# Sh-Anand/Raytracer-in-CPP

Measured on AMD Instinct MI355X. Metric: Mrays/s, higher is better.
Workload: dtype f32; 1 GPU; 1920x1080 depth 4 64-sample area light, cube.obj, 1 light, row stripes of 8 over 1 GPU(s); width=1920, height=1080, max_depth=4, samples=64, scene=cube.obj, parallelism=rows1, step=eager launches

## Files before the change

raytracer-in-cpp_amd/csrc/rt_kernels.hip:

```cpp
#include <hip/hip_runtime.h>

#include <cstdlib>
#include <type_traits>

#include "rt_ao_layout.hpp"
#include "rt_shadow_layout.hpp"
#include "rt_gather_layout.hpp"
#include "rt_probe_layout.hpp"
#include "rt_distance_layout.hpp"
#include "rt_hits_layout.hpp"
#include "rt_device.hpp"
#include "rt_gbuffer_layout.hpp"
#include "rt_launch.hpp"

namespace rtamd {

#define RT_WAVES 4
#define RT_STACK 128

__device__ __forceinline__ float smin(float a, float b) { return (b < a) ? b : a; }
__device__ __forceinline__ float smax(float a, float b) { return (a < b) ? b : a; }
__device__ __forceinline__ float dot3(float ax, float ay, float az, float bx, float by, float bz) {
    return ax * bx + (ay * by + az * bz);
}
__device__ __forceinline__ void normalize3(float &x, float &y, float &z) {
    const float q = x * x + (y * y + z * z);
    if (q > 0.0f) {
        const float s = sqrtf(q);
        x = x / s; y = y / s; z = z / s;
    }
}

#ifdef RT_NO_HOT_LAYOUT
#define RT_LIKELY(x) (x)
#define RT_UNLIKELY(x) (x)
#define RT_SELDOM(x) (x)
#else
#define RT_LIKELY(x) __builtin_expect(static_cast<bool>(x), true)
#define RT_UNLIKELY(x) __builtin_expect(static_cast<bool>(x), false)
#define RT_SELDOM(x) __builtin_expect_with_probability(static_cast<bool>(x), false, 0.97)
#endif

__device__ __forceinline__ void normalize3_fast(const float q, float &x, float &y, float &z) {
    float s = __builtin_amdgcn_sqrtf(q);
    const float sm = __uint_as_float(__float_as_uint(s) - 1u), sp = __uint_as_float(__float_as_uint(s) + 1u);
    const float rm = __builtin_fmaf(-sm, s, q), rp = __builtin_fmaf(-sp, s, q);
    s = rp > 0.0f ? sp : (rm <= 0.0f ? sm : s);
    float r = __builtin_amdgcn_rcpf(s);
    const float e = __builtin_fmaf(-s, r, 1.0f);
    r = __builtin_fmaf(e, r, r);
    float qx = x * r, qy = y * r, qz = z * r;
    qx = __builtin_fmaf(__builtin_fmaf(-s, qx, x), r, qx);
    qy = __builtin_fmaf(__builtin_fmaf(-s, qy, y), r, qy);
    qz = __builtin_fmaf(__builtin_fmaf(-s, qz, z), r, qz);
    x = __builtin_fmaf(__builtin_fmaf(-s, qx, x), r, qx);
    y = __builtin_fmaf(__builtin_fmaf(-s, qy, y), r, qy);
    z = __builtin_fmaf(__builtin_fmaf(-s, qz, z), r, qz);
}
__device__ __forceinline__ void normalize3_shared(float &x, float &y, float &z) {
    const float q = x * x + (y * y + z * z);
    const bool ok = (q >= 0x1p-80f) && (q <= 0x1p80f) && (fminf(fminf(fabsf(x), fabsf(y)), fabsf(z)) >= 0x1p-60f);
    if (RT_LIKELY(__ballot(!ok) == 0ull)) {
        normalize3_fast(q, x, y, z);
    } else if (q > 0.0f) {
        const float s = sqrtf(q);
        x = x / s; y = y / s; z = z / s;
    }
}
template <bool TESTED>
__device__ __forceinline__ void normalize3_shared(const float q, float &x, float &y, float &z) {
    if constexpr (TESTED) {
        normalize3_fast(q, x, y, z);
    } else {
        const bool ok = (q >= 0x1p-80f) && (q <= 0x1p80f) && (fminf(fminf(fabsf(x), fabsf(y)), fabsf(z)) >= 0x1p-60f);
        if (RT_LIKELY(__ballot(!ok) == 0ull)) {
            normalize3_fast(q, x, y, z);
        } else if (q > 0.0f) {
            const float s = sqrtf(q);
            x = x / s; y = y / s; z = z / s;
        }
    }
}

__device__ __forceinline__ uint32_t uniform_u32(uint32_t v) { return __builtin_amdgcn_readfirstlane(v); }
__device__ __forceinline__ unsigned long long uniform_u64(unsigned long long v) {
    const uint32_t lo = __builtin_amdgcn_readfirstlane(static_cast<uint32_t>(v));
    const uint32_t hi = __builtin_amdgcn_readfirstlane(static_cast<uint32_t>(v >> 32));
    return (static_cast<unsigned long long>(hi) << 32) | lo;
}
__device__ __forceinline__ uint32_t lanes_below(unsigned long long m) {
    return __builtin_amdgcn_mbcnt_hi(static_cast<uint32_t>(m >> 32), __builtin_amdgcn_mbcnt_lo(static_cast<uint32_t>(m), 0u));
}

// ... 483 lines not shown
                    RT_PROF_ADD(lane, WORK_TRI_STEPS_LANES_RAYS, 2); RT_PROF_ADD(lane, WORK_TRI_USEFUL_LANES_RAYS, 2 * __popcll(__ballot(mine)));
                    test_lane(ta);
                    test_lane(tb);
                }
                if (k < n) {
                    RT_PROF_ADD(lane, WORK_TRI_STEPS_LANES_RAYS, 1); RT_PROF_ADD(lane, WORK_TRI_USEFUL_LANES_RAYS, __popcll(__ballot(mine)));
                    test_lane(staged[k]);
                }
                if (ANY && !COUNT) {
                    mine = mine && !occluded;
                    if (__ballot(mine) == 0ull) break;
                }
            }
        }
    }
}

template <bool ANY, bool COUNT, bool STAGED = true>
__device__ __forceinline__ auto packet_walk(const DNode *__restrict__ nodes, const TriRec *__restrict__ tris,
                                            const ChunkBound *__restrict__ chunks, const uint32_t *__restrict__ leaf_chunk0,
                                            const float extent, const WaveStack stk, const int lane, const WalkCtl wc, bool in_root, const WalkRay &ray,
                                            uint32_t &cnt_box, uint32_t &cnt_ref, uint32_t &cnt_sig) {
    const RayLane R = make_ray_lane(ray, extent);
    const float ox = R.ox, oy = R.oy, oz = R.oz, idx_ = R.idx, idy_ = R.idy, idz_ = R.idz, slab_pad = R.slab_pad;
    float best_t = 3.402823466e+38f;
    int best_f = -1;
    bool occluded = false;
    int sp = 0;
    {
        unsigned long long m0 = __ballot(in_root);
        if (wc.resume) m0 &= wc.start_mask;
        if (m0 == 0ull) return walk_result<ANY>(best_t, best_f, occluded);
        if (COUNT && in_root && !wc.resume) cnt_box += 1;
        stk.node[0] = wc.resume ? wc.start_node : 0u;
        stk.mask[0] = m0;
        sp = 1;
    }
    while (sp > 0) {
        --sp;
        __builtin_amdgcn_wave_barrier();
        const uint32_t ni = uniform_u32(stk.node[sp]);
        const unsigned long long m = uniform_u64(stk.mask[sp]);
        bool mine = ((m >> lane) & 1ull) != 0ull;
        if (ANY && !COUNT) mine = mine && !occluded;
        unsigned long long live = __ballot(mine);
        if (live == 0ull) continue;
        const DNode nd = nodes[ni];
        const uint32_t cnt = nd.count_flags & 0x7fffffffu;
        if (nd.count_flags & RT_NODE_LEAF) {
            leaf_visit<ANY, COUNT, STAGED>(nd, ni, tris, chunks, leaf_chunk0, stk, lane, wc, R, live, mine, best_t, best_f, occluded, cnt_ref, cnt_sig);
        } else {
            for (uint32_t c = 0; c < cnt; ++c) {
                const uint32_t ci = nd.first + c;
                const DNode ch = nodes[ci];
                bool h = mine;
                if (!COUNT && ch.pad[1] == 0u) {
                    const float t0x = (ch.clo[0] - slab_pad - ox) * idx_, t1x = (ch.chi[0] + slab_pad - ox) * idx_;
                    const float t0y = (ch.clo[1] - slab_pad - oy) * idy_, t1y = (ch.chi[1] + slab_pad - oy) * idy_;
                    const float t0z = (ch.clo[2] - slab_pad - oz) * idz_, t1z = (ch.chi[2] + slab_pad - oz) * idz_;
                    const float tin = fmaxf(fmaxf(fminf(t0x, t1x), fminf(t0y, t1y)), fminf(t0z, t1z));
                    const float tout = fminf(fminf(fmaxf(t0x, t1x), fmaxf(t0y, t1y)), fmaxf(t0z, t1z));
                    const bool miss = (tin > tout) || (tout < -1e-3f) ||
                                      (ANY ? (tin > 0.981f) : (tin > best_t + 1e-3f * (1.0f + fabsf(best_t))));
                    RT_PROF_ADD(lane, WORK_RAY_NODE_PAIRS_CONTENT_CULLED, __popcll(__ballot(h && miss)));
                    h = h && !miss;
                    if (__ballot(h) == 0ull) continue;
                }
                h = h && box_hit_verified(ch.bmin, ox, oy, oz, ray.bx, ray.by, ray.bz, ray.brx, ray.bry, ray.brz);
                RT_PROF_ADD(lane, WORK_BOX_STEPS_STACK_WALK, 1); RT_PROF_ADD(lane, WORK_BOX_USEFUL_STACK_WALK, __popcll(__ballot(mine)));
                if (COUNT && mine) cnt_box += h ? 2u : 1u;
                const unsigned long long hm = __ballot(h);
                if (hm != 0ull) {
                    stk.node[sp] = ci;
                    stk.mask[sp] = hm;
                    ++sp;
                }
            }
        }
    }
    return walk_result<ANY>(best_t, best_f, occluded);
}


template <bool ANY, bool COUNT>
__device__ __forceinline__ auto flat_walk(const DNode &root, const TriRec *__restrict__ tris, bool in_root, const SegPacket &seg, const unsigned long long skip, const LanePlane &pl,
                                          const WalkRay &ray, uint32_t &cnt_box, uint32_t &cnt_ref) {
    const float ox = ray.ox, oy = ray.oy, oz = ray.oz, dx = ray.dx, dy = ray.dy, dz = ray.dz;
    float best_t = 3.402823466e+38f;
    int best_f = -1;
    bool occluded = false;
    if (__ballot(in_root) == 0ull) return walk_result<ANY>(best_t, best_f, occluded);
    const uint32_t cnt = root.count_flags & 0x7fffffffu;
    if (COUNT && in_root) { cnt_box += 1; cnt_ref += cnt; }
    const TriRec *__restrict__ T = tris + root.first;
    bool mine = in_root;
    auto test_one = [&](const TriRec &tr) {
        const float dn = dot3(dx, dy, dz, tr.nx, tr.ny, tr.nz);
        const float t = (tr.nA - dot3(ox, oy, oz, tr.nx, tr.ny, tr.nz)) / dn;
        const float v2x = (ox + t * dx) - tr.ax, v2y = (oy + t * dy) - tr.ay, v2z = (oz + t * dz) - tr.az;
        const float d02 = dot3(tr.e0x, tr.e0y, tr.e0z, v2x, v2y, v2z);
        const float d12 = dot3(tr.e1x, tr.e1y, tr.e1z, v2x, v2y, v2z);
        const float u = (tr.d11 * d02 - tr.d01 * d12) * tr.inv_denom;
        const float v = (tr.d00 * d12 - tr.d01 * d02) * tr.inv_denom;
        const bool ok = mine && !(ANY && (tr.flags & 1u)) && (dn != 0) && (u >= 0) && (v >= 0) && (u + v < 1) && (t > 0.00001f);
        if (ANY) {
            occluded = occluded || (ok && t < 0.98f);
        } else {
            const bool better = ok && (t < best_t || (t == best_t && static_cast<int>(tr.face) < best_f));
            best_t = better ? t : best_t;
            best_f = better ? static_cast<int>(tr.face) : best_f;
        }
    };
    if (ANY && !COUNT && seg.on) {
        unsigned long long keep = low_mask(cnt) & ~skip;
        keep &= ~__ballot(seg.prepared ? plane_rules_out_prepared(seg, pl) : plane_rules_out(seg, pl.nx, pl.ny, pl.nz, pl.nA));
        RT_PROF_ADD(threadIdx.x & 63, WORK_LEAVES_LANES_RAYS, 1); RT_PROF_ADD(threadIdx.x & 63, WORK_TRI_USEFUL_LANES_RAYS, __popcll(keep));
        while (keep != 0ull) {
            const uint32_t k0 = static_cast<uint32_t>(__builtin_ctzll(keep));
            keep &= keep - 1ull;
            if (keep != 0ull) {
                const uint32_t k1 = static_cast<uint32_t>(__builtin_ctzll(keep));
                keep &= keep - 1ull;
                TriRec ta, tb;
                tri_load_uniform_pair(T + k0, T + k1, ta, tb);
                RT_PROF_ADD(threadIdx.x & 63, WORK_TRI_STEPS_LANES_RAYS, 2);
                test_one(ta);
                test_one(tb);
            } else {
                RT_PROF_ADD(threadIdx.x & 63, WORK_TRI_STEPS_LANES_RAYS, 1);
                test_one(tri_load_uniform(T + k0));
            }
            mine = mine && !occluded;
            if (__ballot(mine) == 0ull) break;
        }
        return walk_result<ANY>(best_t, best_f, occluded);
    }
    uint32_t k = 0;
    RT_PROF_ADD(threadIdx.x & 63, WORK_LEAVES_LANES_RAYS, 1);
    for (; k + 1u < cnt; k += 2u) {
        TriRec ta, tb;
        tri_load_uniform2(T + k, ta, tb);
        RT_PROF_ADD(threadIdx.x & 63, WORK_TRI_STEPS_LANES_RAYS, 2);
        test_one(ta);
        test_one(tb);
        if (ANY && !COUNT && (k & 6u) == 6u) {
            mine = mine && !occluded;
            if (__ballot(mine) == 0ull) return walk_result<ANY>(best_t, best_f, occluded);
        }
    }
    if (k < cnt) { RT_PROF_ADD(threadIdx.x & 63, WORK_TRI_STEPS_LANES_RAYS, 1); test_one(tri_load_uniform(T + k)); }
    return walk_result<ANY>(best_t, best_f, occluded);
}

template <bool ANY, bool COUNT, bool FLAT, bool STAGED = true>
__device__ __forceinline__ auto walk(const DNode &root, const DNode *__restrict__ nodes, const TriRec *__restrict__ tris,
                                     const ChunkBound *__restrict__ chunks, const uint32_t *__restrict__ leaf_chunk0,
                                     const float extent, const WaveStack stk, const int lane, const WalkCtl wc, const LanePlane &pl, bool in_root,
                                     const WalkRay &ray, uint32_t &cnt_box, uint32_t &cnt_ref) {
    uint32_t sig_unused = 0u;
    if constexpr (FLAT) return flat_walk<ANY, COUNT>(root, tris, in_root, wc.seg, wc.skip, pl, ray, cnt_box, cnt_ref);
    else return packet_walk<ANY, COUNT, STAGED>(nodes, tris, chunks, leaf_chunk0, extent, stk, lane, wc, in_root, ray, cnt_box, cnt_ref, sig_unused);
}

template <bool COUNT>
__device__ __forceinline__ bool flat_unit_occluded(const DNode &root, const TriRec *__restrict__ tris, const SegPacket &seg, const unsigned long long skip,
                                                   const LanePlane &pl, const bool valid, const WalkRay &ray, uint32_t &cnt_box, uint32_t &cnt_ref) {
    return flat_walk<true, COUNT>(root, tris, valid && root_hit(root, ray), seg, skip, pl, ray, cnt_box, cnt_ref);
}

#ifndef RT_SHAFT_TRUNC
#define RT_SHAFT_TRUNC 0.0185f
#endif
struct ShaftLanes {
    float r[8];
    float pad;
    bool node_ok;
};

__device__ __forceinline__ ShaftLanes make_shaft_lanes(const int lane, const float hx, const float hy, const float hz, const float slx, const float sly,
                                                       const float slz, const float shx, const float shy, const float shz, const float extent,
                                                       const float trunc = 0.0f) {
    ShaftLanes SL;
    const int tk = lane & 7, proj = tk >> 1;
    const bool q1 = (tk & 1) != 0;
    const float big = fmaxf(fmaxf(fabsf(slx), fabsf(shx)), fmaxf(fabsf(sly), fabsf(shy))) + fmaxf(fabsf(slz), fabsf(shz));
    const float scale = extent + big + (fabsf(hx) + fabsf(hy) + fabsf(hz));
    SL.pad = 4e-4f * ((fmaxf(fabsf(slx), fabsf(shx)) + fmaxf(fabsf(sly), fabsf(shy)) + fmaxf(fabsf(slz), fabsf(shz))) + extent) * 1.001f;
    SL.node_ok = true;
    const float hu = proj == 1 ? hy : hx, hv = proj == 2 ? hy : hz;
    const float u0 = proj == 1 ? sly : slx, u1 = proj == 1 ? shy : shx;
    const float v0 = proj == 2 ? sly : slz, v1 = proj == 2 ? shy : shz;
    const bool ul = hu < u0, ur = hu > u1, vl = hv < v0, vr = hv > v1;
    const bool su0 = !(ul || ur), sv0 = !(vl || vr);
    const float near_u = ul ? u0 : u1, far_u = ul ? u1 : u0, near_v = vl ? v0 : v1, far_v = vl ? v1 : v0;
    const float cu = q1 ? (su0 ? u1 : (sv0 ? near_u : far_u)) : (su0 ? u0 : near_u);
    const float cv = q1 ? (sv0 ? v1 : near_v) : (sv0 ? v0 : (su0 ? near_v : far_v));
    const float mu = 0.5f * (u0 + u1) - hu, mv = 0.5f * (v0 + v1) - hv;
    const float nu = -(cv - hv), nv = cu - hu;
    const float fm = nu * mu + nv * mv;
    const float mag = fabsf(nu) + fabsf(nv);
    const bool ok = !(su0 && sv0) && (fabsf(fm) > 1e-5f * mag * scale);
    const float sgn = fm > 0.0f ? -1.0f : 1.0f;
    const float a = ok ? sgn * nu : 0.0f, b = ok ? sgn * nv : 0.0f;
    const float margin = 2e-5f * mag * scale;
    const float c = ok ? -(a * hu + b * hv) - margin : -1.0f;
    const float ax = proj == 1 ? 0.0f : a, ay = proj == 0 ? 0.0f : (proj == 1 ? a : b), az = proj == 2 ? 0.0f : b;
    SL.r[0] = fmaxf(ax, 0.0f); SL.r[1] = fminf(ax, 0.0f); SL.r[2] = fmaxf(ay, 0.0f); SL.r[3] = fminf(ay, 0.0f);
    SL.r[4] = fmaxf(az, 0.0f); SL.r[5] = fminf(az, 0.0f); SL.r[6] = c; SL.r[7] = ok ? 2.0f * margin : 3e38f;
    if (tk == 6) {
        SL.r[0] = fminf(slx, hx); SL.r[1] = fminf(sly, hy); SL.r[2] = fminf(slz, hz);
        SL.r[3] = fmaxf(shx, hx); SL.r[4] = fmaxf(shy, hy); SL.r[5] = fmaxf(shz, hz);
        if (trunc > 0.0f) {
            const float m = 1e-5f * scale;
            SL.r[0] += hx < slx ? fmaxf(trunc * (slx - hx) - m, 0.0f) : 0.0f; SL.r[3] -= hx > shx ? fmaxf(trunc * (hx - shx) - m, 0.0f) : 0.0f;
            SL.r[1] += hy < sly ? fmaxf(trunc * (sly - hy) - m, 0.0f) : 0.0f; SL.r[4] -= hy > shy ? fmaxf(trunc * (hy - shy) - m, 0.0f) : 0.0f;
            SL.r[2] += hz < slz ? fmaxf(trunc * (slz - hz) - m, 0.0f) : 0.0f; SL.r[5] -= hz > shz ? fmaxf(trunc * (hz - shz) - m, 0.0f) : 0.0f;
        }
    }
    if (tk == 7) {
        SL.r[0] = hx >= shx ? hx : -3e38f; SL.r[1] = hy >= shy ? hy : -3e38f; SL.r[2] = hz >= shz ? hz : -3e38f;
        SL.r[3] = hx <= slx ? hx : 3e38f; SL.r[4] = hy <= sly ? hy : 3e38f; SL.r[5] = hz <= slz ? hz : 3e38f;
    }
    return SL;
}

__device__ __forceinline__ void shaft_lane_test(const ShaftLanes &SL, const int tk, const float lx, const float ly, const float lz, const float hx, const float hy,
                                                const float hz, bool &near_out, bool &far_out, const bool near_box = true) {
    const float mn = __builtin_fmaf(SL.r[0], lx, __builtin_fmaf(SL.r[1], hx, __builtin_fmaf(SL.r[2], ly, __builtin_fmaf(SL.r[3], hy,
                     __builtin_fmaf(SL.r[4], lz, __builtin_fmaf(SL.r[5], hz, SL.r[6]))))));
    const float mx = __builtin_fmaf(SL.r[0], hx, __builtin_fmaf(SL.r[1], lx, __builtin_fmaf(SL.r[2], hy, __builtin_fmaf(SL.r[3], ly,
                     __builtin_fmaf(SL.r[4], hz, __builtin_fmaf(SL.r[5], lz, SL.r[6]))))));
    const bool box_out = (lx > SL.r[3]) || (hx < SL.r[0]) || (ly > SL.r[4]) || (hy < SL.r[1]) || (lz > SL.r[5]) || (hz < SL.r[2]);
    near_out = tk < 6 ? (mn > 0.0f) : (tk == 6 && near_box && box_out);
// ... 691 lines not shown
    r.lx = it.lx; r.ly = it.ly; r.lz = it.lz; r.lmode = it.lmode; r.pix = it.pix;
    r.pre = r.valid;
    return r;
}
template <bool PRIMARY, bool LENS, bool SHUTTER, bool PASS>
__device__ __forceinline__ TileRay tile_ray(const uint32_t tile, const int lane, const DFrame &F, const DCam &cam, const DShutter &shut, const DNode &root,
                                            const RayItem *__restrict__ rays_in, const ShardMap &rmap) {
    if (PRIMARY) {
        uint32_t pt = tile;
        unsigned long long lanes = ~0ull;
        if (F.tiles != nullptr) flag_tile(F, rmap, tile, pt, lanes);
        return primary_ray<LENS, SHUTTER, PASS>(pt, lanes, lane, F, cam, shut, root);
    }
    return listed_ray(tile, lane, F, rays_in, rmap);
}

__device__ __forceinline__ void finish_tile(const TileRay &r, const bool hit, const bool lit, const int best_f, const float best_t, const uint32_t tile,
                                            const int level, const int lane, const DFrame &F, ShadeItem *__restrict__ items, Control *__restrict__ ctl,
                                            float4 *__restrict__ rec, int32_t *__restrict__ out_hit, float *__restrict__ out_t) {
    if (r.valid) {
        if (!hit) rec[r.pix] = background_record();
        else if (!lit) rec[r.pix] = shadow_record();
        if (out_hit) out_hit[r.pix] = hit ? best_f : -1;
        if (out_t) out_t[r.pix] = hit ? best_t : -1.0f;
    }
    const unsigned long long lm = __ballot(lit);
    if (lm != 0ull) {
        bool fits;
        const uint32_t base = shard_reserve(ctl->n_items[level], &ctl->overflow, tile, static_cast<uint32_t>(__popcll(lm)), F.item_cap, lane, fits);
        if (lit && fits) {
            ShadeItem o;
            o.ox = r.ox; o.oy = r.oy; o.oz = r.oz; o.dx = r.dx; o.dy = r.dy; o.dz = r.dz;
            o.lx = r.lx; o.ly = r.ly; o.lz = r.lz; o.lmode = r.lmode; o.pix = r.pix; o.face = best_f; o.t = best_t;
            o.pad0 = o.pad1 = o.pad2 = 0u;
            items[base + lanes_below(lm)] = o;
        }
    }
}
template <bool PRIMARY, bool COUNT>
__device__ __forceinline__ void flush_trace_counters(Control *__restrict__ ctl, const int lane, const int level, uint32_t c_rays, uint32_t c_cull,
                                                     uint32_t c_centre, uint32_t c_box, uint32_t c_ref, const uint32_t c_outside) {
    c_rays = wave_sum(c_rays); c_cull = wave_sum(c_cull); c_centre = wave_sum(c_centre);
    c_cull += c_outside;
    if (COUNT) { c_box = wave_sum(c_box); c_ref = wave_sum(c_ref); }
    if (lane == 0) {
        if (c_rays) stat_add(ctl, (PRIMARY || level == 0) ? ST_RAYS_PRIMARY : ST_RAYS_BOUNCE, c_rays);
        if (c_cull) stat_add(ctl, ST_PIXELS_CULLED, c_cull);
        if (c_centre) stat_add(ctl, ST_RAYS_CENTRE, c_centre);
        if (COUNT) {
            if (c_box) stat_add(ctl, ST_BOX_TESTS, c_box);
            if (c_ref) stat_add(ctl, ST_LEAF_TRI_REFS, c_ref);
        }
    }
}

template <bool COUNT, bool FLAT>
__device__ __forceinline__ bool centre_lit(const DNode &root, const DNode *__restrict__ nodes, const TriRec *__restrict__ tris, const ChunkBound *__restrict__ chunks,
                                           const uint32_t *__restrict__ leaf_chunk0, const float extent, const WaveStack stk, const int lane, const DLights &L,
                                           const bool hit, const float hx, const float hy, const float hz, const uint32_t lmode, const float lx, const float ly,
                                           const float lz, uint32_t &c_centre, uint32_t &c_box, uint32_t &c_ref) {
    bool lit = false;
    const int nl_lane = lmode ? 1 : L.n_lights;
    const int nl_wave = (__ballot(hit && lmode == 0u) != 0ull) ? L.n_lights : 1;
    if (__ballot(hit) != 0ull) {
        for (int l = 0; l < nl_wave; ++l) {
            const bool act = hit && (l < nl_lane);
            float px, py, pz;
            light_point(L, l, lmode, lx, ly, lz, px, py, pz);
            c_centre += act ? 1u : 0u;
            if (COUNT && act) c_box += 1;
            const WalkRay ray = segment_ray(px, py, pz, hx, hy, hz);
            const bool occ = walk<true, COUNT, FLAT>(root, nodes, tris, chunks, leaf_chunk0, extent, stk, lane, walk_plain(), LanePlane{}, act && root_hit(root, ray), ray,
                                                     c_box, c_ref);
            lit = lit || (act && !occ);
        }
    }
    return lit;
}
__device__ __forceinline__ Hit flat_closest_hit(const DNode &root, const TriRec *__restrict__ tris, const bool active, const float ox, const float oy, const float oz,
                                                const float dx, const float dy, const float dz) {
    const WalkRay ray = trace_ray(ox, oy, oz, dx, dy, dz);
    uint32_t cu0 = 0, cu1 = 0;
    return flat_walk<false, false>(root, tris, active && root_hit(root, ray), seg_off(), 0ull, LanePlane{}, ray, cu0, cu1);
}

template <bool PRIMARY, bool COUNT, bool FLAT, bool LENS = false, bool SHUTTER = false, bool PASS = false>
__global__ __launch_bounds__(RT_WAVES * 64) void k_trace(const DNode *__restrict__ nodes, const TriRec *__restrict__ tris,
                                                          const ChunkBound *__restrict__ chunks, const uint32_t *__restrict__ leaf_chunk0,
                                                          const DScene S, const CamArg camarg, const DLights L, const DFrame F,
                                                          const int level, const int ctr_slot,
                                                          const RayItem *__restrict__ rays_in, ShadeItem *__restrict__ items,
                                                          Control *__restrict__ ctl, float4 *__restrict__ rec,
                                                          int32_t *__restrict__ out_hit, float *__restrict__ out_t) {
    __shared__ uint4 s_stage[FLAT ? 1 : RT_WAVES * RT_STAGE_TRIS * 5];
    __shared__ unsigned long long s_mask[FLAT ? 1 : RT_WAVES * RT_STACK];
    __shared__ uint32_t s_node[FLAT ? 1 : RT_WAVES * RT_STACK];
    const int lane = threadIdx.x & 63, wave = threadIdx.x >> 6;
    const WaveStack stk{s_node + (FLAT ? 0 : wave * RT_STACK), s_mask + (FLAT ? 0 : wave * RT_STACK), s_stage + (FLAT ? 0 : wave * RT_STAGE_TRIS * 5)};
    ShardMap rmap{0u, 0u, 0u, 0u};
    if (!PRIMARY) rmap = shard_map(ctl->n_rays[level], lane, 0xffffffffu, 1u, 64u);
    else if (F.tiles != nullptr) rmap = shard_map(ctl->n_flag, lane, F.tile_cap, 1u, 1u);
    uint32_t ntiles = (!PRIMARY || F.tiles != nullptr) ? rmap.total : static_cast<uint32_t>(F.tiles_x) * static_cast<uint32_t>(F.tiles_y);
    if (!PRIMARY && ntiles == 0u) return;
    const DNode root = nodes[0];
    DCam cam;
    if (PRIMARY) cam = cam_of(camarg);
    DShutter shut;
    if (PRIMARY && SHUTTER) shut = shutter_of(camarg);
    constexpr bool CULL = PRIMARY && !COUNT && !LENS && !SHUTTER && !PASS;
    const bool cull = CULL && F.cull != 0;
    CullRect crect{0, 0, 0, 0};
    bool window = false;
    uint32_t wx0 = 0, wy0 = 0, ww = 1, c_outside = 0;
    if (cull) {
        crect = cull_rect(camarg);
        if (F.nranks == 1 && out_hit == nullptr && out_t == nullptr) {
            window = true;
            const int lx0 = crect.x0 < F.width ? crect.x0 : F.width, lx1 = crect.x1 < F.width ? crect.x1 : F.width;
            int ly0 = crect.y0 - F.row0, ly1 = crect.y1 - F.row0;
            ly0 = ly0 < 0 ? 0 : (ly0 < F.local_rows ? ly0 : F.local_rows);
            ly1 = ly1 < 0 ? 0 : (ly1 < F.local_rows ? ly1 : F.local_rows);
            ntiles = 0u; c_outside = F.npix;
            if (lx0 < lx1 && ly0 < ly1) {
                const int wx1 = (lx1 + 7) / 8, wy1 = (ly1 + 7) / 8;
                wx0 = static_cast<uint32_t>(lx0 / 8); wy0 = static_cast<uint32_t>(ly0 / 8);
                ww = static_cast<uint32_t>(wx1) - wx0;
                ntiles = ww * (static_cast<uint32_t>(wy1) - wy0);
                const int px1 = wx1 * 8 < F.width ? wx1 * 8 : F.width, py1 = wy1 * 8 < F.local_rows ? wy1 * 8 : F.local_rows;
                c_outside = F.npix - static_cast<uint32_t>(px1 - static_cast<int>(wx0) * 8) * static_cast<uint32_t>(py1 - static_cast<int>(wy0) * 8);
            }
        }
    }

    uint32_t c_rays = 0, c_cull = 0, c_centre = 0, c_box = 0, c_ref = 0;
    ShardedQueue q;
    if (F.dyn_trace) q.init(ctl->queue[ctr_slot], ntiles, gridDim.x * RT_WAVES, blockIdx.x, lane);
    else q.init_static(ntiles, gridDim.x * RT_WAVES, uniform_u32(blockIdx.x * RT_WAVES + static_cast<uint32_t>(wave)), lane);
    for (uint32_t tile = 0; q.next(tile);) {
        RT_PROF_ADD(lane, WORK_UNITS, 1);
        TileRay r;
        if (PRIMARY) {
            uint32_t pt = tile;
            unsigned long long lanes = ~0ull;
            if (F.tiles != nullptr) flag_tile(F, rmap, tile, pt, lanes);
            if (window) pt = (wy0 + tile / ww) * static_cast<uint32_t>(F.tiles_x) + wx0 + tile % ww;
            if (cull && !window) {
                const int tx = static_cast<int>(pt % static_cast<uint32_t>(F.tiles_x)), ty = static_cast<int>(pt / static_cast<uint32_t>(F.tiles_x));
                if (tile_outside(F, crect, tx, ty)) {
                    const int x = tx * 8 + (lane & 7), lr = ty * 8 + (lane >> 3);
                    const bool valid = (x < F.width) && (lr < F.local_rows) && ((lanes >> lane) & 1ull) != 0ull;
                    const uint32_t pix = static_cast<uint32_t>(lr) * static_cast<uint32_t>(F.width) + static_cast<uint32_t>(x);
                    c_cull += valid ? 1u : 0u;
                    if (valid && out_hit) out_hit[pix] = -1;
                    if (valid && out_t) out_t[pix] = -1.0f;
                    continue;
                }
            }
            r = primary_ray<LENS, SHUTTER, PASS>(pt, lanes, lane, F, cam, shut, root);
            c_cull += (r.valid && !r.pre) ? 1u : 0u;
        } else {
            r = listed_ray(tile, lane, F, rays_in, rmap);
        }
        bool in_root = r.pre;
        c_rays += in_root ? 1u : 0u;
        const WalkRay ray = trace_ray(r.ox, r.oy, r.oz, r.dx, r.dy, r.dz);
        if (COUNT && in_root) c_box += 1;
        in_root = in_root && root_hit(root, ray);

        const Hit best = walk<false, COUNT, FLAT>(root, nodes, tris, chunks, leaf_chunk0, S.extent, stk, lane, walk_plain(), LanePlane{}, in_root, ray, c_box, c_ref);
        const bool hit = r.valid && found(best.face, S.n_faces);
        const float hx = r.ox + best.t * r.dx, hy = r.oy + best.t * r.dy, hz = r.oz + best.t * r.dz;
        const bool lit = centre_lit<COUNT, FLAT>(root, nodes, tris, chunks, leaf_chunk0, S.extent, stk, lane, L, hit, hx, hy, hz, r.lmode, r.lx, r.ly, r.lz,
                                                 c_centre, c_box, c_ref);

        finish_tile(r, hit, lit, best.face, best.t, tile, level, lane, F, items, ctl, rec, out_hit, out_t);
    }
    flush_trace_counters<PRIMARY, COUNT>(ctl, lane, level, c_rays, c_cull, c_centre, c_box, c_ref, (CULL && blockIdx.x == 0 && wave == 0) ? c_outside : 0u);
}


#define RT_NO_HIT_KEY 0xffffffffffffffffull

template <bool PRIMARY, bool COUNT, int STAGE, bool CONT, bool LENS = false, bool SHUTTER = false, bool PASS = false>
__global__ __launch_bounds__(RT_WAVES * 64) void k_stage(const DNode *__restrict__ nodes, const TriRec *__restrict__ tris,
                                                          const ChunkBound *__restrict__ chunks, const uint32_t *__restrict__ leaf_chunk0,
                                                          const DScene S, const CamArg camarg, const DLights L, const DFrame F,
                                                          const int level, const int lslots,
                                                          const RayItem *__restrict__ rays_in, ShadeItem *__restrict__ items,
                                                          Control *__restrict__ ctl, float4 *__restrict__ rec,
                                                          int32_t *__restrict__ out_hit, float *__restrict__ out_t,
                                                          unsigned long long *best, unsigned long long *lit, const TaskQueues Q) {
    constexpr bool CONE = CONT && STAGE < 2 && !COUNT;
    __shared__ uint4 s_stage[RT_WAVES * RT_STAGE_TRIS * 5];
    __shared__ unsigned long long s_mask[RT_WAVES * RT_STACK];
    __shared__ uint32_t s_node[RT_WAVES * RT_STACK];
    __shared__ float4 s_cone[CONE ? RT_WAVES * RT_SHAFT_TRI_REC : 1];
    const int lane = threadIdx.x & 63, wave = threadIdx.x >> 6;
    const WaveStack stk{s_node + wave * RT_STACK, s_mask + wave * RT_STACK, s_stage + wave * RT_STAGE_TRIS * 5};
    float4 *const cone_rec = s_cone + (CONE ? wave * RT_SHAFT_TRI_REC : 0);
    ShardMap rmap{0u, 0u, 0u, 0u};
    if (!PRIMARY) rmap = shard_map(ctl->n_rays[level], lane, 0xffffffffu, 1u, 64u);
    else if (F.tiles != nullptr) rmap = shard_map(ctl->n_flag, lane, F.tile_cap, 1u, 1u);
    const uint32_t ntiles = (!PRIMARY || F.tiles != nullptr) ? rmap.total : static_cast<uint32_t>(F.tiles_x) * static_cast<uint32_t>(F.tiles_y);

    uint32_t n_units = STAGE == 1 ? ntiles * static_cast<uint32_t>(lslots) : ntiles;
    ShardMap tmap{0u, 0u, 0u, 0u};
    if (CONT) {
        tmap = shard_map(ctl->n_task_tr[level][Q.q_in & 1u], lane, Q.cap / RT_LIST_SHARDS, 1u, 1u);
        n_units = tmap.total;
    }
    if (n_units == 0u) return;
    const DNode root = nodes[0];
    DCam cam;
    if (PRIMARY) cam = cam_of(camarg);
    DShutter shut;
    if (PRIMARY && SHUTTER) shut = shutter_of(camarg);
    constexpr bool CULL = PRIMARY && !COUNT && !CONT && !LENS && !SHUTTER && !PASS;
    const bool cull = CULL && F.cull != 0;
    CullRect crect{0, 0, 0, 0};
    if (cull) crect = cull_rect(camarg);

    uint32_t c_rays = 0, c_cull = 0, c_centre = 0, c_box = 0, c_ref = 0;
    ShardedQueue q;
    q.init_static(n_units, gridDim.x * RT_WAVES, uniform_u32(blockIdx.x * RT_WAVES + static_cast<uint32_t>(wave)), lane);
    for (uint32_t work = 0; q.next(work);) {
        uint32_t unit = work;
        WalkCtl wc = walk_plain();
        RT_PROF_ADD(lane, WORK_UNITS, 1);
        if (CONT) {
            uint32_t tsh, tloc, tn;
            shard_find(tmap, work, tsh, tloc, tn);
            const ContTask task = Q.tasks_in[tsh * (Q.cap / RT_LIST_SHARDS) + tloc];
            unit = uniform_u32(task.unit);
            wc.resume = true;
            wc.start_node = uniform_u32(task.node);
            wc.start_mask = uniform_u64(task.mask);
            wc.c_begin = uniform_u32(task.c_begin);
            wc.c_end = uniform_u32(task.c_end);
        }
        if (STAGE < 2 && Q.tasks_out != nullptr && Q.budget != 0u) {
            const uint32_t tsh = blockIdx.x & (RT_LIST_SHARDS - 1u), tcap = Q.cap / RT_LIST_SHARDS;
            wc.budget = Q.budget; wc.unit = unit; wc.tasks = Q.tasks_out + tsh * tcap; wc.task_count = &ctl->n_task_tr[level][Q.q_out & 1u][tsh * 16u]; wc.task_cap = tcap;
            wc.target = Q.target ? Q.target : Q.budget;
        }
        const uint32_t tile = STAGE == 1 ? unit / static_cast<uint32_t>(lslots) : unit;
        const int l = STAGE == 1 ? static_cast<int>(unit - tile * static_cast<uint32_t>(lslots)) : 0;
        if (cull) {
            const int tx = static_cast<int>(tile % static_cast<uint32_t>(F.tiles_x)), ty = static_cast<int>(tile / static_cast<uint32_t>(F.tiles_x));
            if (tile_outside(F, crect, tx, ty)) {
                const int x = tx * 8 + (lane & 7), lr = ty * 8 + (lane >> 3);
                const bool valid = (x < F.width) && (lr < F.local_rows);
                if (STAGE == 0) c_cull += valid ? 1u : 0u;
                if (STAGE == 2 && valid) {
                    const uint32_t pix = static_cast<uint32_t>(lr) * static_cast<uint32_t>(F.width) + static_cast<uint32_t>(x);
                    if (out_hit) out_hit[pix] = -1;
                    if (out_t) out_t[pix] = -1.0f;
// ... 378 lines not shown
        shard_find(imap, unit, sh, lu, n_sh);
        const uint32_t g = P == 1u ? lu : udiv(lu, P, inv_P, sh_P), pass = lu - g * P;
        const uint32_t item_i = lslots == 1 ? g : udiv(g, static_cast<uint32_t>(lslots), inv_ls, sh_ls);
        const int l = static_cast<int>(g - item_i * static_cast<uint32_t>(lslots));
        uint32_t item_at = uniform_u32(sh * item_cap + item_i);
        if (sidx != nullptr) item_at = uniform_u32(sidx[item_at]);
        if (!CONT && Q.pair_done != nullptr) {
            const size_t di = static_cast<size_t>(item_at) * static_cast<size_t>(lslots) + static_cast<size_t>(l);
            const uint32_t dw = reinterpret_cast<const uint32_t *>(Q.pair_done)[di >> 2];
            if (((dw >> (8u * static_cast<uint32_t>(di & 3u))) & 0xffu) != 0u) continue;
        }
        const ShadeItem it = items[item_at];
        uint32_t s = pass * 64u + static_cast<uint32_t>(lane);
        float fi = fi_lane + 0.5f, fj = fj_lane + 0.5f;
        float b_i0 = 0.5f, b_j0 = 0.5f, b_i1 = fi_last, b_j1 = fj_last;
        if (blocks) {
            const uint32_t bi = udiv(pass, bpr, inv_bpr, sh_bpr), bj = pass - bi * bpr;
            s = (bi * 8u + (static_cast<uint32_t>(lane) >> 3)) * vst + bj * 8u + (static_cast<uint32_t>(lane) & 7u);
            b_i0 = static_cast<float>(bi * 8u) + 0.5f; b_j0 = static_cast<float>(bj * 8u) + 0.5f;
            b_i1 = static_cast<float>(bi * 8u + 7u) + 0.5f; b_j1 = static_cast<float>(bj * 8u + 7u) + 0.5f;
            fi = (static_cast<float>(bi * 8u) + fi_lane) + 0.5f; fj = (static_cast<float>(bj * 8u) + fj_lane) + 0.5f;
        } else if (P > 1u) {
            fi = static_cast<float>(s / vst) + 0.5f; fj = static_cast<float>(s % vst) + 0.5f;
        }
        const int nl = it.lmode ? 1 : L.n_lights;
        const bool valid = s < N && l < nl;
        float hx, hy, hz;
        hit_point(it, hx, hy, hz);
        LightGrid lg = lg0;
        if (it.lmode != 0u || l != 0) {
            float px, py, pz;
            light_point(L, l, it.lmode, it.lx, it.ly, it.lz, px, py, pz);
            lg = light_grid(L, px, py, pz);
        }
        float sx, sy, sz, x0, y0, z0, x1, y1, z1;
        grid_sample(lg, fi, fj, sx, sy, sz);
        grid_sample(lg, b_i0, b_j0, x0, y0, z0);
        grid_sample(lg, b_i1, b_j1, x1, y1, z1);
        if (L.mode == RT_LIGHT_SPHERE) {
            float px, py, pz;
            light_point(L, l, it.lmode, it.lx, it.ly, it.lz, px, py, pz);
            sphere_sample(L, s, px, py, pz, sx, sy, sz);
            sphere_box(L, px, py, pz, x0, y0, z0, x1, y1, z1);
        }
        const WalkRay ray = segment_ray(sx, sy, sz, hx, hy, hz);
        const unsigned long long vis_index = (static_cast<unsigned long long>(item_at) * static_cast<unsigned long long>(lslots) + static_cast<unsigned long long>(l)) * P + pass;
        if (!CONT) c_rays += static_cast<uint32_t>(__popcll(__ballot(valid)));
        ShaftLanes SL = make_shaft_lanes(lane, hx, hy, hz, fminf(x0, x1), fminf(y0, y1), fminf(z0, z1), fmaxf(x0, x1), fmaxf(y0, y1), fmaxf(z0, z1), S.extent, RT_SHAFT_TRUNC);
        __builtin_amdgcn_wave_barrier();
        shaft_tri_store(sl.tri, lane, SL, hx, hy, hz, fminf(x0, x1), fminf(y0, y1), fminf(z0, z1), fmaxf(x0, x1), fmaxf(y0, y1), fmaxf(z0, z1));
        shaft_lanes_store(sl.shaft, lane, SL);
        __builtin_amdgcn_wave_barrier();
        ShaftCtl SC{SL.pad, true};
        SC.node_ok = __ballot(valid && !(fabsf(ray.dx) > 0.0f && fabsf(ray.dy) > 0.0f && fabsf(ray.dz) > 0.0f && fabsf(ray.dx) + fabsf(ray.dy) + fabsf(ray.dz) < 3e38f)) == 0ull;
        const RayLane R = make_ray_lane(ray, S.extent);
        bool occ = false;
        const bool tasks_on = TASKS && Q.tasks_out != nullptr && Q.budget != 0u && units < 256u * gridDim.x * RT_WAVES;
        const uint32_t tsh = blockIdx.x & (RT_LIST_SHARDS - 1u), tcap = Q.cap / RT_LIST_SHARDS;
        if (CONT) {
            const ShaftTasks TQ{nullptr, nullptr, 0u, 0u, 0u, unit};
            const unsigned long long live = t_mask & uniform_u64(vis[vis_index]);
            if (live != 0ull) {
                const DNode leaf = nodes[t_node];
                shaft_leaf<false>(t_node, uniform_u32(leaf.first), uniform_u32(leaf.count_flags) & 0x7fffffffu, uniform_u32(leaf.pad[0]), tris, chunks, lane, R, SC, TQ,
                           sl, t_cb, t_ce, live, occ);
            }
            const unsigned long long om = __ballot(valid && occ);
            if (lane == 0 && om != 0ull) atomicAnd(&vis[vis_index], ~om);
        } else {
            const DNode rootl = sl.nodes[0];
            const bool sroot = valid && root_hit(rootl, ray);
            const ShaftTasks TQ{Q.tasks_out + tsh * tcap, &ctl->n_task_sh[level][tsh * 16u], tcap, tasks_on ? Q.budget : 0u, Q.target ? Q.target : Q.budget, unit};
            shaft_walk<TASKS>(nodes, tris, chunks, stk, sl, lane, rootl, sroot, R, SC, TQ, occ);
            const unsigned long long vm = __ballot(valid && !occ);
            if (lane == 0) vis[vis_index] = vm;
        }
    }
    if (lane == 0 && c_rays) {
        stat_add(ctl, ST_RAYS_SAMPLE, c_rays);
        stat_add(ctl, ST_SAMPLE_WALKED, c_rays);
    }
}

__device__ __forceinline__ bool plane_rules_out_box(const float slx, const float sly, const float slz, const float shx, const float shy, const float shz,
                                                    const float hlx, const float hly, const float hlz, const float hhx, const float hhy, const float hhz,
                                                    const float m0, const float nx, const float ny, const float nz, const float nA) {
    const float ax = nx * slx, bx = nx * shx, ay = ny * sly, by = ny * shy, az = nz * slz, bz = nz * shz;
    const float sn_lo = fminf(ax, bx) + (fminf(ay, by) + fminf(az, bz));
    const float sn_hi = fmaxf(ax, bx) + (fmaxf(ay, by) + fmaxf(az, bz));
    const float cx = nx * hlx, dx = nx * hhx, cy = ny * hly, dy = ny * hhy, cz = nz * hlz, dz = nz * hhz;
    const float hn_lo = fminf(cx, dx) + (fminf(cy, dy) + fminf(cz, dz));
    const float hn_hi = fmaxf(cx, dx) + (fmaxf(cy, dy) + fmaxf(cz, dz));
    const float num_lo = nA - sn_hi, num_hi = nA - sn_lo;
    const float dn_lo = hn_lo - sn_hi, dn_hi = hn_hi - sn_lo;
    const float M = m0 + 2e-5f * fabsf(nA);
    const bool sane = (fabsf(nx) + fabsf(ny) + fabsf(nz) <= 4.0f) && (fabsf(nA) <= 1e30f);
    const bool opposite = (num_lo > M && dn_hi < -M) || (num_hi < -M && dn_lo > M);
    const float min_abs_num = fmaxf(num_lo, -num_hi);
    const float max_abs_dn = fmaxf(fabsf(dn_lo), fabsf(dn_hi));
    const bool beyond = (min_abs_num - M) >= 0.981f * (max_abs_dn + M);
    const float e_max = fmaxf(fabsf(hn_lo - nA), fabsf(hn_hi - nA));
    const float a_min = min_abs_num - M;
    const bool near_plane = (a_min > 0.0f) && (e_max + 2.0f * M <= 0.018f * a_min);
    return sane && (num_lo <= num_hi) && (dn_lo <= dn_hi) && (hn_lo <= hn_hi) && (opposite || beyond || near_plane);
}
__device__ __forceinline__ void shaft_inflate(ShaftLanes &SL, const int tk, const float ex, const float ey, const float ez) {
    if (tk < 6) {
        const float ax = SL.r[0] + SL.r[1], ay = SL.r[2] + SL.r[3], az = SL.r[4] + SL.r[5];
        SL.r[6] = SL.r[6] - ((fabsf(ax) * ex + fabsf(ay) * ey) + fabsf(az) * ez) * 1.0001f;
    } else if (tk == 6) {
        SL.r[0] -= ex; SL.r[1] -= ey; SL.r[2] -= ez; SL.r[3] += ex; SL.r[4] += ey; SL.r[5] += ez;
    }
}
struct ItemPlane { float a, b, c, far_margin; };
template <int PROJ, bool Q1>
__device__ __forceinline__ ItemPlane item_plane(const float hx, const float hy, const float hz, const float slx, const float sly, const float slz,
                                                const float shx, const float shy, const float shz, const float scale) {
    const float hu = PROJ == 1 ? hy : hx, hv = PROJ == 2 ? hy : hz;
    const float u0 = PROJ == 1 ? sly : slx, u1 = PROJ == 1 ? shy : shx;
    const float v0 = PROJ == 2 ? sly : slz, v1 = PROJ == 2 ? shy : shz;
    const bool ul = hu < u0, ur = hu > u1, vl = hv < v0, vr = hv > v1;
    const bool su0 = !(ul || ur), sv0 = !(vl || vr);
    const float near_u = ul ? u0 : u1, far_u = ul ? u1 : u0, near_v = vl ? v0 : v1, far_v = vl ? v1 : v0;
    const float cu = Q1 ? (su0 ? u1 : (sv0 ? near_u : far_u)) : (su0 ? u0 : near_u);
    const float cv = Q1 ? (sv0 ? v1 : near_v) : (sv0 ? v0 : (su0 ? near_v : far_v));
    const float mu = 0.5f * (u0 + u1) - hu, mv = 0.5f * (v0 + v1) - hv;
    const float nu = -(cv - hv), nv = cu - hu;
    const float fm = nu * mu + nv * mv;
    const float mag = fabsf(nu) + fabsf(nv);
    const bool ok = !(su0 && sv0) && (fabsf(fm) > 1e-5f * mag * scale);
    const float sgn = fm > 0.0f ? -1.0f : 1.0f;
    const float margin = 2e-5f * mag * scale;
    ItemPlane p;
    p.a = ok ? sgn * nu : 0.0f; p.b = ok ? sgn * nv : 0.0f;
    p.c = ok ? -(p.a * hu + p.b * hv) - margin : -1.0f;
    p.far_margin = ok ? 2.0f * margin : 3e38f;
    return p;
}
template <int PROJ>
__device__ __forceinline__ void item_plane_test(const ItemPlane &p, const float lx, const float ly, const float lz, const float hx, const float hy, const float hz,
                                                bool &near_out, bool &far_out) {
    const float ul = PROJ == 1 ? ly : lx, uh = PROJ == 1 ? hy : hx, vl = PROJ == 2 ? ly : lz, vh = PROJ == 2 ? hy : hz;
    const float ap = fmaxf(p.a, 0.0f), an = fminf(p.a, 0.0f), bp = fmaxf(p.b, 0.0f), bn = fminf(p.b, 0.0f);
    const float mn = __builtin_fmaf(ap, ul, __builtin_fmaf(an, uh, __builtin_fmaf(bp, vl, __builtin_fmaf(bn, vh, p.c))));
    const float mx = __builtin_fmaf(ap, uh, __builtin_fmaf(an, ul, __builtin_fmaf(bp, vh, __builtin_fmaf(bn, vl, p.c))));
    near_out = near_out || (mn > 0.0f);
    far_out = far_out || (mx + p.far_margin < 0.0f);
}

#ifndef RT_BEAM_BUDGET
#define RT_BEAM_BUDGET 1024
#endif
#ifndef RT_PAIR_WPE
#define RT_PAIR_WPE 6
#endif
#define RT_BEAM_REC 13

__device__ __forceinline__ bool tri_outside_beam(const float4 *rec, const TriRec &tr, const float m) {
    if (tri_outside_cone(rec, tr, m, true)) return true;
    const float4 hm = rec[8], s0 = rec[9], s1 = rec[10], h0 = rec[11], h1 = rec[12];
    return plane_rules_out_box(s0.x, s0.y, s0.z, s1.x, s1.y, s1.z, h0.x, h0.y, h0.z, h1.x, h1.y, h1.z, hm.w, tr.nx, tr.ny, tr.nz, tr.nA);
}

__device__ __forceinline__ bool beam_leaf(const uint32_t first, const uint32_t cnt, const uint32_t chunk0, const TriRec *__restrict__ tris,
                                          const ChunkBound *__restrict__ chunks, const int lane, const float4 *shaft, const float4 *rec, const ShaftCtl &SC,
                                          const bool per_item, int &budget) {
    const TriRec *__restrict__ T = tris + first;
    const ChunkBound *__restrict__ cbounds = chunks + chunk0;
    const uint32_t nchunk = (cnt + 63u) >> 6;
    const int tk = lane & 7, tc = lane >> 3;
    for (uint32_t cb0 = 0u; cb0 < nchunk; cb0 += 8u) {
        const uint32_t myc = cb0 + static_cast<uint32_t>(tc);
        const ChunkBound bd = cbounds[myc < nchunk ? myc : cb0];
        const ShaftLanes SL = shaft_lanes_load(shaft, tk, SC);
        bool near_out, far_out;
        shaft_lane_test(SL, tk, bd.lo[0], bd.lo[1], bd.lo[2], bd.hi[0], bd.hi[1], bd.hi[2], near_out, far_out);
        const unsigned long long b_out = __ballot(near_out && bd.never < 1.5f);
        const uint32_t nhere = nchunk - cb0 < 8u ? nchunk - cb0 : 8u;
        unsigned long long cm = __ballot(static_cast<uint32_t>(lane) < nhere && !ballot_byte_any(b_out, lane));
        const unsigned long long nv = __ballot(static_cast<uint32_t>(lane) < nhere && ((cm >> lane) & 1ull) != 0ull && __shfl(bd.never, 8 * (lane & 7), 64) >= 1.5f);
        if (nv != 0ull && !per_item) return true;
        cm &= ~nv;
        budget -= 1 + static_cast<int>(__popcll(cm));
        RT_PROF_ADD(lane, WORK_BEAM_CHUNK_BATCHES, 1); RT_PROF_ADD(lane, WORK_BEAM_CHUNKS_TESTED_BY_TRIANGLE, __popcll(cm)); if (cb0 == 0u) RT_PROF_ADD(lane, WORK_BEAM_LEAF_VISITS, 1);
        if (budget < 0) return true;
        while (cm != 0ull) {
            const int j = static_cast<int>(__builtin_ctzll(cm));
            cm &= cm - 1ull;
// ... 2904 lines not shown
```

Measured before the change: 219,900 Mrays/s.

## Cull centre shadow triangles per wave and share ray-plane numerators across lanes

```diff
diff --git a/raytracer-in-cpp_amd/csrc/rt_kernels.hip b/raytracer-in-cpp_amd/csrc/rt_kernels.hip
--- a/raytracer-in-cpp_amd/csrc/rt_kernels.hip
+++ b/raytracer-in-cpp_amd/csrc/rt_kernels.hip
@@ -9,6 +9,7 @@
 #include "rt_probe_layout.hpp"
 #include "rt_distance_layout.hpp"
 #include "rt_hits_layout.hpp"
+#include "rt_plane_rule.hpp"
 #include "rt_device.hpp"
 #include "rt_gbuffer_layout.hpp"
 #include "rt_launch.hpp"
@@ -658,9 +659,9 @@
 }
 
 
-template <bool ANY, bool COUNT>
+template <bool ANY, bool COUNT, bool NUM = false>
 __device__ __forceinline__ auto flat_walk(const DNode &root, const TriRec *__restrict__ tris, bool in_root, const SegPacket &seg, const unsigned long long skip, const LanePlane &pl,
-                                          const WalkRay &ray, uint32_t &cnt_box, uint32_t &cnt_ref) {
+                                          const WalkRay &ray, uint32_t &cnt_box, uint32_t &cnt_ref, const float lane_num = 0.0f) {
     const float ox = ray.ox, oy = ray.oy, oz = ray.oz, dx = ray.dx, dy = ray.dy, dz = ray.dz;
     float best_t = 3.402823466e+38f;
     int best_f = -1;
@@ -670,9 +671,12 @@
     if (COUNT && in_root) { cnt_box += 1; cnt_ref += cnt; }
     const TriRec *__restrict__ T = tris + root.first;
     bool mine = in_root;
-    auto test_one = [&](const TriRec &tr) {
+    auto test_one = [&](const TriRec &tr, const uint32_t k_tri) {
         const float dn = dot3(dx, dy, dz, tr.nx, tr.ny, tr.nz);
-        const float t = (tr.nA - dot3(ox, oy, oz, tr.nx, tr.ny, tr.nz)) / dn;
+        float num;
+        if constexpr (NUM) num = __int_as_float(__builtin_amdgcn_readlane(__float_as_int(lane_num), static_cast<int>(k_tri)));
+        else num = tr.nA - dot3(ox, oy, oz, tr.nx, tr.ny, tr.nz);
+        const float t = num / dn;
         const float v2x = (ox + t * dx) - tr.ax, v2y = (oy + t * dy) - tr.ay, v2z = (oz + t * dz) - tr.az;
         const float d02 = dot3(tr.e0x, tr.e0y, tr.e0z, v2x, v2y, v2z);
         const float d12 = dot3(tr.e1x, tr.e1y, tr.e1z, v2x, v2y, v2z);
@@ -700,11 +704,11 @@
                 TriRec ta, tb;
                 tri_load_uniform_pair(T + k0, T + k1, ta, tb);
                 RT_PROF_ADD(threadIdx.x & 63, WORK_TRI_STEPS_LANES_RAYS, 2);
-                test_one(ta);
-                test_one(tb);
+                test_one(ta, k0);
+                test_one(tb, k1);
             } else {
                 RT_PROF_ADD(threadIdx.x & 63, WORK_TRI_STEPS_LANES_RAYS, 1);
-                test_one(tri_load_uniform(T + k0));
+                test_one(tri_load_uniform(T + k0), k0);
             }
             mine = mine && !occluded;
             if (__ballot(mine) == 0ull) break;
@@ -717,14 +721,14 @@
         TriRec ta, tb;
         tri_load_uniform2(T + k, ta, tb);
         RT_PROF_ADD(threadIdx.x & 63, WORK_TRI_STEPS_LANES_RAYS, 2);
-        test_one(ta);
-        test_one(tb);
+        test_one(ta, k);
+        test_one(tb, k + 1u);
         if (ANY && !COUNT && (k & 6u) == 6u) {
             mine = mine && !occluded;
             if (__ballot(mine) == 0ull) return walk_result<ANY>(best_t, best_f, occluded);
         }
     }
-    if (k < cnt) { RT_PROF_ADD(threadIdx.x & 63, WORK_TRI_STEPS_LANES_RAYS, 1); test_one(tri_load_uniform(T + k)); }
+    if (k < cnt) { RT_PROF_ADD(threadIdx.x & 63, WORK_TRI_STEPS_LANES_RAYS, 1); test_one(tri_load_uniform(T + k), k); }
     return walk_result<ANY>(best_t, best_f, occluded);
 }
 
@@ -1582,6 +1586,50 @@
     const WalkRay ray = trace_ray(ox, oy, oz, dx, dy, dz);
     uint32_t cu0 = 0, cu1 = 0;
     return flat_walk<false, false>(root, tris, active && root_hit(root, ray), seg_off(), 0ull, LanePlane{}, ray, cu0, cu1);
+}
+
+#ifdef RT_NO_TRACE_CENTRE_CULL
+#define RT_TRACE_CENTRE_CULL false
+#else
+#define RT_TRACE_CENTRE_CULL true
+#endif
+#ifdef RT_NO_TRACE_SHARED_NUM
+#define RT_TRACE_SHARED_NUM false
+#else
+#define RT_TRACE_SHARED_NUM true
+#endif
+__device__ __forceinline__ LanePlane lane_plane_none() { return LanePlane{0.f, 0.f, 0.f, 3e38f, 0.f, 0.f}; }
+template <bool SHARE>
+__device__ __forceinline__ bool trace_centre_lit(const DNode &root, const TriRec *__restrict__ tris, const DScene &S, const int lane, const DLights &L,
+                                                 const LanePlane &tpl, const bool hit, const float hx, const float hy, const float hz, const uint32_t lmode,
+                                                 const float lx, const float ly, const float lz, uint32_t &c_centre) {
+    uint32_t cu0 = 0, cu1 = 0;
+    if (S.plane_cull == 0 || __ballot(hit && lmode != 0u) != 0ull)
+        return centre_lit<false, true>(root, nullptr, tris, nullptr, nullptr, S.extent, WaveStack{nullptr, nullptr, nullptr}, lane, L, hit, hx, hy, hz, lmode, lx, ly, lz,
+                                       c_centre, cu0, cu1);
+    if (__ballot(hit) == 0ull) return false;
+    float blx = hit ? hx : 3e38f, bly = hit ? hy : 3e38f, blz = hit ? hz : 3e38f;
+    float bux = hit ? hx : -3e38f, buy = hit ? hy : -3e38f, buz = hit ? hz : -3e38f;
+#pragma unroll
+    for (int o = 32; o > 0; o >>= 1) {
+        blx = fminf(blx, __shfl_xor(blx, o, 64)); bly = fminf(bly, __shfl_xor(bly, o, 64)); blz = fminf(blz, __shfl_xor(blz, o, 64));
+        bux = fmaxf(bux, __shfl_xor(bux, o, 64)); buy = fmaxf(buy, __shfl_xor(buy, o, 64)); buz = fmaxf(buz, __shfl_xor(buz, o, 64));
+    }
+    SegPacket seg = seg_off();
+    seg.on = true;
+    bool lit = false;
+    for (int l = 0; l < L.n_lights; ++l) {
+        const float px = L.pos[l][0], py = L.pos[l][1], pz = L.pos[l][2];
+        c_centre += hit ? 1u : 0u;
+        const WalkRay ray = segment_ray(px, py, pz, hx, hy, hz);
+        const float m0 = plane_rule_m0(px, py, pz, px, py, pz, blx, bly, blz, bux, buy, buz);
+        const unsigned long long skip = __ballot(plane_rules_out_box(px, py, pz, px, py, pz, blx, bly, blz, bux, buy, buz, m0, tpl.nx, tpl.ny, tpl.nz, tpl.nA));
+        float num = 0.0f;
+        if constexpr (SHARE) num = tpl.nA - dot3(px, py, pz, tpl.nx, tpl.ny, tpl.nz);
+        const bool occ = flat_walk<true, false, SHARE>(root, tris, hit && root_hit(root, ray), seg, skip, lane_plane_none(), ray, cu0, cu1, num);
+        lit = lit || (hit && !occ);
+    }
+    return lit;
 }
 
 template <bool PRIMARY, bool COUNT, bool FLAT, bool LENS = false, bool SHUTTER = false, bool PASS = false>
@@ -1632,6 +1680,20 @@
         }
     }
 
+    constexpr bool CENTRE_CULL = FLAT && !COUNT && RT_TRACE_CENTRE_CULL;
+    constexpr bool SHARE_NUM = FLAT && !COUNT && RT_TRACE_SHARED_NUM;
+    constexpr bool CAM_NUM = SHARE_NUM && PRIMARY && !LENS && !SHUTTER;
+    LanePlane tpl = lane_plane_none();
+    float cam_num = 0.0f;
+    if constexpr (CENTRE_CULL || CAM_NUM) {
+        const uint32_t fcnt = root.count_flags & 0x7fffffffu;
+        if (static_cast<uint32_t>(lane) < fcnt) {
+            const TriRec &tk = tris[root.first + static_cast<uint32_t>(lane)];
+            tpl.nx = tk.nx; tpl.ny = tk.ny; tpl.nz = tk.nz; tpl.nA = tk.nA;
+        }
+        if constexpr (CAM_NUM) cam_num = tpl.nA - dot3(cam.center[0], cam.center[1], cam.center[2], tpl.nx, tpl.ny, tpl.nz);
+    }
+
     uint32_t c_rays = 0, c_cull = 0, c_centre = 0, c_box = 0, c_ref = 0;
     ShardedQueue q;
     if (F.dyn_trace) q.init(ctl->queue[ctr_slot], ntiles, gridDim.x * RT_WAVES, blockIdx.x, lane);
@@ -1667,11 +1729,15 @@
         if (COUNT && in_root) c_box += 1;
         in_root = in_root && root_hit(root, ray);
 
-        const Hit best = walk<false, COUNT, FLAT>(root, nodes, tris, chunks, leaf_chunk0, S.extent, stk, lane, walk_plain(), LanePlane{}, in_root, ray, c_box, c_ref);
+        Hit best;
+        if constexpr (CAM_NUM) best = flat_walk<false, false, true>(root, tris, in_root, seg_off(), 0ull, LanePlane{}, ray, c_box, c_ref, cam_num);
+        else best = walk<false, COUNT, FLAT>(root, nodes, tris, chunks, leaf_chunk0, S.extent, stk, lane, walk_plain(), LanePlane{}, in_root, ray, c_box, c_ref);
         const bool hit = r.valid && found(best.face, S.n_faces);
         const float hx = r.ox + best.t * r.dx, hy = r.oy + best.t * r.dy, hz = r.oz + best.t * r.dz;
-        const bool lit = centre_lit<COUNT, FLAT>(root, nodes, tris, chunks, leaf_chunk0, S.extent, stk, lane, L, hit, hx, hy, hz, r.lmode, r.lx, r.ly, r.lz,
-                                                 c_centre, c_box, c_ref);
+        bool lit;
+        if constexpr (CENTRE_CULL) lit = trace_centre_lit<SHARE_NUM>(root, tris, S, lane, L, tpl, hit, hx, hy, hz, r.lmode, r.lx, r.ly, r.lz, c_centre);
+        else lit = centre_lit<COUNT, FLAT>(root, nodes, tris, chunks, leaf_chunk0, S.extent, stk, lane, L, hit, hx, hy, hz, r.lmode, r.lx, r.ly, r.lz,
+                                           c_centre, c_box, c_ref);
 
         finish_tile(r, hit, lit, best.face, best.t, tile, level, lane, F, items, ctl, rec, out_hit, out_t);
     }
@@ -2216,28 +2282,6 @@
     }
 }
 
-__device__ __forceinline__ bool plane_rules_out_box(const float slx, const float sly, const float slz, const float shx, const float shy, const float shz,
-                                                    const float hlx, const float hly, const float hlz, const float hhx, const float hhy, const float hhz,
-                                                    const float m0, const float nx, const float ny, const float nz, const float nA) {
-    const float ax = nx * slx, bx = nx * shx, ay = ny * sly, by = ny * shy, az = nz * slz, bz = nz * shz;
-    const float sn_lo = fminf(ax, bx) + (fminf(ay, by) + fminf(az, bz));
-    const float sn_hi = fmaxf(ax, bx) + (fmaxf(ay, by) + fmaxf(az, bz));
-    const float cx = nx * hlx, dx = nx * hhx, cy = ny * hly, dy = ny * hhy, cz = nz * hlz, dz = nz * hhz;
-    const float hn_lo = fminf(cx, dx) + (fminf(cy, dy) + fminf(cz, dz));
-    const float hn_hi = fmaxf(cx, dx) + (fmaxf(cy, dy) + fmaxf(cz, dz));
-    const float num_lo = nA - sn_hi, num_hi = nA - sn_lo;
-    const float dn_lo = hn_lo - sn_hi, dn_hi = hn_hi - sn_lo;
-    const float M = m0 + 2e-5f * fabsf(nA);
-    const bool sane = (fabsf(nx) + fabsf(ny) + fabsf(nz) <= 4.0f) && (fabsf(nA) <= 1e30f);
-    const bool opposite = (num_lo > M && dn_hi < -M) || (num_hi < -M && dn_lo > M);
-    const float min_abs_num = fmaxf(num_lo, -num_hi);
-    const float max_abs_dn = fmaxf(fabsf(dn_lo), fabsf(dn_hi));
-    const bool beyond = (min_abs_num - M) >= 0.981f * (max_abs_dn + M);
-    const float e_max = fmaxf(fabsf(hn_lo - nA), fabsf(hn_hi - nA));
-    const float a_min = min_abs_num - M;
-    const bool near_plane = (a_min > 0.0f) && (e_max + 2.0f * M <= 0.018f * a_min);
-    return sane && (num_lo <= num_hi) && (dn_lo <= dn_hi) && (hn_lo <= hn_hi) && (opposite || beyond || near_plane);
-}
 __device__ __forceinline__ void shaft_inflate(ShaftLanes &SL, const int tk, const float ex, const float ey, const float ez) {
     if (tk < 6) {
         const float ax = SL.r[0] + SL.r[1], ay = SL.r[2] + SL.r[3], az = SL.r[4] + SL.r[5];
diff --git a/raytracer-in-cpp_amd/csrc/rt_plane_rule.hpp b/raytracer-in-cpp_amd/csrc/rt_plane_rule.hpp
--- /dev/null
+++ b/raytracer-in-cpp_amd/csrc/rt_plane_rule.hpp
@@ -0,0 +1,37 @@
+#pragma once
+
+#include <cmath>
+
+#include "rt_query_chunks.hpp"
+
+namespace rtamd {
+
+RT_QUERY_HD bool plane_rules_out_box(const float slx, const float sly, const float slz, const float shx, const float shy, const float shz,
+                                     const float hlx, const float hly, const float hlz, const float hhx, const float hhy, const float hhz,
+                                     const float m0, const float nx, const float ny, const float nz, const float nA) {
+    const float ax = nx * slx, bx = nx * shx, ay = ny * sly, by = ny * shy, az = nz * slz, bz = nz * shz;
+    const float sn_lo = fminf(ax, bx) + (fminf(ay, by) + fminf(az, bz));
+    const float sn_hi = fmaxf(ax, bx) + (fmaxf(ay, by) + fmaxf(az, bz));
+    const float cx = nx * hlx, dx = nx * hhx, cy = ny * hly, dy = ny * hhy, cz = nz * hlz, dz = nz * hhz;
+    const float hn_lo = fminf(cx, dx) + (fminf(cy, dy) + fminf(cz, dz));
+    const float hn_hi = fmaxf(cx, dx) + (fmaxf(cy, dy) + fmaxf(cz, dz));
+    const float num_lo = nA - sn_hi, num_hi = nA - sn_lo;
+    const float dn_lo = hn_lo - sn_hi, dn_hi = hn_hi - sn_lo;
+    const float M = m0 + 2e-5f * fabsf(nA);
+    const bool sane = (fabsf(nx) + fabsf(ny) + fabsf(nz) <= 4.0f) && (fabsf(nA) <= 1e30f);
+    const bool opposite = (num_lo > M && dn_hi < -M) || (num_hi < -M && dn_lo > M);
+    const float min_abs_num = fmaxf(num_lo, -num_hi);
+    const float max_abs_dn = fmaxf(fabsf(dn_lo), fabsf(dn_hi));
+    const bool beyond = (min_abs_num - M) >= 0.981f * (max_abs_dn + M);
+    const float e_max = fmaxf(fabsf(hn_lo - nA), fabsf(hn_hi - nA));
+    const float a_min = min_abs_num - M;
+    const bool near_plane = (a_min > 0.0f) && (e_max + 2.0f * M <= 0.018f * a_min);
+    return sane && (num_lo <= num_hi) && (dn_lo <= dn_hi) && (hn_lo <= hn_hi) && (opposite || beyond || near_plane);
+}
+RT_QUERY_HD float plane_rule_m0(const float slx, const float sly, const float slz, const float shx, const float shy, const float shz,
+                                const float hlx, const float hly, const float hlz, const float hhx, const float hhy, const float hhz) {
+    return 2e-5f * (((fabsf(slx) + fabsf(shx)) + (fabsf(sly) + fabsf(shy)) + (fabsf(slz) + fabsf(shz))) +
+                    ((fabsf(hlx) + fabsf(hhx)) + (fabsf(hly) + fabsf(hhy)) + (fabsf(hlz) + fabsf(hhz))));
+}
+
+}
```

New measurement: 221,800 Mrays/s (median of 6 runs). No clear change (+0.8%).
